# ChainBreak/denoising_diffusion_deep_fake

Hardware: AMD Instinct MI355X
Metric: training images/sec (256x256 U-Net, bs=16/GPU) (higher is better)
Workload: dtype f32; 1 GPU; d3f train_denoiser step: noise blend -> Unet(resnet34) fwd -> (MSE+1-SSIM)/2 -> bwd -> Adam, 256x256 synthetic face crops, bs=16/GPU, random-init weights, train-mode BatchNorm; image_size=256, batch_per_gpu=16, global_batch=16, parallelism=dp1, graph_step=False, adam_overlap_tail=False, adam_overlap_tail_steps=0, ranks_seen=1, csrc_digest=7380406eeae80552

## Files before the change

### denoising_diffusion_deep_fake_amd/csrc/common.h

```cpp
#pragma once
#include <hip/hip_runtime.h>
#include <stdint.h>
#include <stddef.h>
#include <stdlib.h>

namespace d3f {

typedef uint16_t bf16_t;

typedef float f32x16 __attribute__((ext_vector_type(16)));
typedef float f32x4 __attribute__((ext_vector_type(4)));
typedef __bf16 bf16x8 __attribute__((ext_vector_type(8)));

}
#ifndef D3F_F32
#define D3F_F32 0
#define D3F_BF16 1
#define D3F_F32X3 2
#endif
namespace d3f {

static inline const char* prof_knob(const char* name) {
#ifdef D3F_PROFILING
  return getenv(name);
// ... 168 lines not shown
  unsigned div_howo_mul, div_howo_shr, div_wo_mul, div_wo_shr;
  int cin_real;
  int sum2;
  int patch;
  int nets, plan_nets;
  long net_ws, net_out0, net_scale;
  int tile_bm, tile_bn;
};
__device__ __forceinline__ ConvParams conv_params_of_net(const ConvParams& pin, int net) {
  ConvParams p = pin;
  if (net != 0) {
    net_shift(p.src0, p.net_ws); net_shift(p.src1, p.net_ws); net_shift(p.w, p.net_ws);
    net_shift(p.out0, p.net_out0); net_shift(p.out1, p.net_ws);
    net_shift(p.stats, p.net_ws); net_shift(p.scale, p.net_scale); net_shift(p.shift, p.net_ws);
    net_shift(p.res, p.net_ws); net_shift(p.partial, p.net_ws);
    net_shift(p.bn_y, p.net_ws); net_shift(p.bn_coef, p.net_ws); net_shift(p.bn_partial, p.net_ws); net_shift(p.bn_a, p.net_ws);
  }
  return p;
}

struct ConvTile {
  int BM, BN;
};
int conv_igemm_plan(ConvParams& p, int dtype, bool allow_splitk = false);
size_t conv_splitk_floats(const ConvParams& p);
int conv_igemm_launch(const ConvParams& p, int dtype, hipStream_t stream);
bool conv_igemm_small_c(const ConvParams& p, int dtype);
bool conv_igemm_fast_addr(const ConvParams& p, bool smallc);
bool conv_winograd_fits(const ConvParams& p, int dtype);
bool conv_winograd_applies(const ConvParams& p, int dtype);
int conv_winograd_stat_rows(const ConvParams& p);
size_t conv_winograd_filter_floats(const ConvParams& p);
int conv_winograd_pack_launch(const float* w , float* u, int Cout, int Cin, hipStream_t stream);
int conv_winograd_launch(const ConvParams& p , hipStream_t stream);
bool conv_pres_applies(const ConvParams& p, int dtype);
void conv_pres_plan(ConvParams& p);
int conv_pres_launch(const ConvParams& p, hipStream_t stream);
bool conv_patch_applies(const ConvParams& p, int dtype);
bool conv_stem_applies(const ConvParams& p, int dtype);
bool conv_stem_bf16_applies(const ConvParams& p, int dtype);
void conv_patch_plan(ConvParams& p, int dtype);
int conv_patch_launch(const ConvParams& p, hipStream_t stream);

struct WgradParams {
  const void* dy;
  const void* src0;
  const void* src1;
  float* partial;
  unsigned dy_bytes, src0_bytes, src1_bytes;
  int B, Hv, Wv, C0, C1, H0s, W0s, shift0;
  int Ho, Wo, Cout;
  int KH, KW, stride, pad;
  int M;
  int cin_real;
  int splits;
  int chunks_per_split;
  int tiles_co, tiles_ci;
  int patch;
  double flops;
  int part;
  int cls;
  int ci_base;
  int slab_cin;
  int slab_taps;
  int Mi, Hc, Wc;
  int step_img, step_row, step_col;
// ... 106 lines not shown
```

### denoising_diffusion_deep_fake_amd/csrc/conv_winograd.hip

```cpp
#include "common.h"

#include <cstdlib>

namespace d3f {

namespace {
constexpr int WCK = 16;
constexpr int WPP = 18;
constexpr int WPB = 4;
typedef float wf32x2 __attribute__((ext_vector_type(2)));

__device__ __forceinline__ int vsw(int row, int ch) { return ch ^ ((row >> 2) & 3); }
}

bool conv_winograd_fits(const ConvParams& p, int dtype) {
  if (dtype != D3F_F32) return false;
  if (p.mode != CONV_RAW_STATS || p.par != 0 || p.KH != 3 || p.KW != 3 || p.stride != 1 || p.pad != 1 || p.C1 != 0 ||
      p.shift0 != 0 || p.zi != 0 || p.Ho != p.Hv || p.Wo != p.Wv || (p.Ho % 16) != 0 || (p.Wo % 16) != 0 ||
      (p.C0 % WCK) != 0 || (p.Cout % 64) != 0 || p.CoutPad < p.Cout)
    return false;
  if ((size_t)p.B * p.Hv * p.Wv * p.C0 * 4 >= (1ull << 31) || (size_t)16 * p.C0 * p.Cout * 4 >= (1ull << 31)) return false;
  return (long)p.B * (p.Ho / 16) * (p.Wo / 16) * (p.Cout / 64) <= 65535L * 4;
}
bool conv_winograd_applies(const ConvParams& p, int dtype) {
  static const bool off = getenv("D3F_NO_WINOGRAD") != nullptr;
  if (off || !conv_winograd_fits(p, dtype)) return false;
  const long wgs = (long)p.B * (p.Ho / 16) * (p.Wo / 16) * (p.Cout / 64) * plan_nets_for(p.plan_nets, 8);
  return wgs >= 256;
}
int conv_winograd_stat_rows(const ConvParams& p) { return p.B * (p.Ho / 16) * (p.Wo / 16); }
size_t conv_winograd_filter_floats(const ConvParams& p) { return (size_t)16 * p.C0 * p.Cout; }

__global__ __launch_bounds__(256) void winograd_pack_kernel(const float* __restrict__ w, float* __restrict__ u, int K, int C) {
  const int id = (int)blockIdx.x * 256 + (int)threadIdx.x;
  if (id >= K * C) return;
  const int k = id / C, c = id - k * C;
  const float* g = w + (long)id * 9;
  float t[4][3];
#pragma unroll
  for (int j = 0; j < 3; ++j) {
    const float g0 = g[j], g1 = g[3 + j], g2 = g[6 + j];
    t[0][j] = g0;
    t[1][j] = 0.5f * (g0 + g1 + g2);
    t[2][j] = 0.5f * (g0 - g1 + g2);
    t[3][j] = g2;
  }
  const long cstride = (long)(C / WCK) * K * WCK;
  float* dst = u + ((long)(c / WCK) * K + k) * WCK + (c % WCK);
#pragma unroll
  for (int i = 0; i < 4; ++i) {
    dst[(4 * i + 0) * cstride] = t[i][0];
    dst[(4 * i + 1) * cstride] = 0.5f * (t[i][0] + t[i][1] + t[i][2]);
    dst[(4 * i + 2) * cstride] = 0.5f * (t[i][0] - t[i][1] + t[i][2]);
    dst[(4 * i + 3) * cstride] = t[i][2];
  }
}

int conv_winograd_pack_launch(const float* w, float* u, int K, int C, hipStream_t stream) {
  D3F_CHECK((C % WCK) == 0 && K > 0 && C > 0, "winograd pack: %d filters x %d channels", K, C);
  hipLaunchKernelGGL(winograd_pack_kernel, dim3((unsigned)cdiv((long)K * C, 256)), dim3(256), 0, stream, w, u, K, C);
  D3F_HIP(hipGetLastError());
  return 0;
}

__global__ __launch_bounds__(256) void conv_winograd_kernel(const ConvParams pin) {
  chain_priority();
  const ConvParams p = conv_params_of_net(pin, (int)blockIdx.z);
  __shared__ __attribute__((aligned(16))) float P[WPP * WPP * WCK];
  __shared__ __attribute__((aligned(16))) float V[2][16 * 64 * WCK];
  const int H = p.Hv, W = p.Wv, C = p.C0, K = p.Cout;
  const int tid = threadIdx.x, lane = tid & 63, wave = tid >> 6;
  const int mt = wave >> 1, nt = wave & 1;
  const int bx = W / 16, by = H / 16;
  const int blk = blockIdx.x;
  const int x0 = (blk % bx) * 16, y0 = ((blk / bx) % by) * 16, b = blk / (bx * by);
  const int n0 = blockIdx.y * 64;
  const __amdgpu_buffer_rsrc_t rx = make_rsrc(p.src0, p.src0_bytes);
  const __amdgpu_buffer_rsrc_t ru = make_rsrc(p.w, p.w_bytes);

  f32x16 acc[16];
#pragma unroll
  for (int q = 0; q < 16; ++q)
#pragma unroll
    for (int r = 0; r < 16; ++r) acc[q][r] = 0.f;

  constexpr int NPX = (WPP * WPP * 4 + 255) / 256;
  uint4 px[NPX];
  unsigned poff[NPX];
#pragma unroll
  for (int i = 0; i < NPX; ++i) {
    const int id = tid + 256 * i, pix = id >> 2, h = id & 3;
    const int py = pix / WPP, pxx = pix - py * WPP;
    const int gy = y0 - 1 + py, gx = x0 - 1 + pxx;
    const bool ok = id < WPP * WPP * 4 && (unsigned)gy < (unsigned)H && (unsigned)gx < (unsigned)W;
    poff[i] = ok ? (unsigned)((((b * H + gy) * W + gx) * C + 4 * h) * 4) : BUF_OOB;
// ... 188 lines not shown
```

### denoising_diffusion_deep_fake_amd/csrc/engine.hip

```cpp
#include "engine.h"
#include <vector>

#include "head_act.h"

#include <cstdio>
#include <cstdlib>
#include <cstring>

namespace d3f {

constexpr int CS_PP = 16;
__global__ __launch_bounds__(256) void channel_sum_partial_kernel(const float* __restrict__ x, int C, long HW,
                                                                  float* __restrict__ partial, int nb, long net_in,
                                                                  long net_ws) {
  __shared__ float red[256];
  const int seg = blockIdx.x, c = blockIdx.y, b = (int)blockIdx.z % nb;
  if ((int)blockIdx.z >= nb) {
    net_shift(x, net_in); net_shift(partial, net_ws);
  }
  const float* __restrict__ plane = x + ((long)b * C + c) * HW;
  const long per = (HW + CS_PP - 1) / CS_PP, lo = (long)seg * per, hi = lo + per < HW ? lo + per : HW;
  float s = 0.f;
  if ((HW & 3) == 0 && (per & 3) == 0) {
    for (long i = lo + 4 * threadIdx.x; i < hi; i += 4 * 256) {
// ... 391 lines not shown
  if (streams[dev] == nullptr) {
    int least = 0, greatest = 0;
    D3F_HIP(hipDeviceGetStreamPriorityRange(&least, &greatest));
    D3F_HIP(hipStreamCreateWithPriority(&streams[dev], hipStreamNonBlocking, least));
  }
  *out = streams[dev];
  return 0;
}

int UnetEngine::ensure_streams() const {
  if (side_ != nullptr) return 0;
  if (int rc = shared_side_stream(&side_)) return rc;
  D3F_HIP(hipEventCreateWithFlags(&ev_join_, hipEventDisableTiming));
  D3F_HIP(hipEventCreateWithFlags(&ev_seg_, hipEventDisableTiming));
  D3F_HIP(hipEventCreateWithFlags(&ev_pack_in_, hipEventDisableTiming));
  D3F_HIP(hipEventCreateWithFlags(&ev_pack_done_, hipEventDisableTiming));
  D3F_HIP(hipEventCreateWithFlags(&ev_pack_mid_, hipEventDisableTiming));
  return 0;
}

bool UnetEngine::make_split(const NetIO* io, long in_delta, NetSplit* ns) const {
  if (nets <= 1) return false;
  ns->nets = nets;
  ns->ws = (long)net_ws_stride;
  ns->par = io->params;
  ns->grad = io->grads;
  ns->bn = io->bnstats;
  ns->in = in_delta;
  ns->out = io->out;
  return true;
}

int UnetEngine::pack_weights(const float* params0_, void* ws0_, hipStream_t s, const NetIO* io) const {
  D3F_CHECK((int)units.size() <= PACK_MAX_LAYERS, "pack_weights: %d layers exceed the table", (int)units.size());
  D3F_CHECK(nets == 1 || io != nullptr, "pack_weights: a pair engine needs the second network's offsets");
  static const bool sync_pack = getenv("D3F_NO_ASYNC_PACK") != nullptr;
  const bool async = !sync_pack && first_late_unit_ > 0;
  const int mid = async ? first_mid_unit_ : -1;
  auto params_of = [&](int n) { return reinterpret_cast<const float*>(reinterpret_cast<const char*>(params0_) + (n ? io->params : 0)); };
  auto ws_of = [&](int n) { return reinterpret_cast<char*>(ws0_) + (size_t)n * net_ws_stride; };
  auto part_of = [&](int ui) { return ui >= first_late_unit_ ? 2 : (mid > 0 && ui >= mid) ? 1 : 0; };
  for (int part = 0; part < 3; ++part) {
    if (part == 1 && mid <= 0) continue;
    PackTable t;
    t.n = 0;
    uint32_t blocks = 0;
    for (int ui = 0; ui < (int)units.size(); ++ui) {
      const Unit& u = units[ui];
      if (first_late_unit_ > 0 && part_of(ui) != part) continue;
      if (first_late_unit_ <= 0 && part != 0) continue;
      if (u.upfold) continue;
      const int nb = conv_pack_entry(u, u.w_off, u.wf_off, u.wd_off, true, u.need_dgrad, blocks, t.e[t.n++]);
      if (nb < 0) return nb;
      blocks += (uint32_t)nb;
    }
    hipStream_t ps = s;
    if (part >= 1 && async) {
      if (int rc = ensure_streams()) return rc;
      if (part == 1 || mid <= 0) {
        D3F_HIP(hipEventRecord(ev_pack_in_, s));
        D3F_HIP(hipStreamWaitEvent(side_, ev_pack_in_, 0));
      }
      ps = side_;
    }
    for (int n = 0; n < nets; ++n) {
      const float* params_ = params_of(n);
      char* ws = ws_of(n);
      if (t.n > 0)
        if (int rc = pack_all_launch(cdtype, params_, ws, t, (int)blocks, ps)) return rc;
      for (int ui = 0; ui < (int)units.size(); ++ui) {
        const Unit& u = units[ui];
        if (!u.wino) continue;
        if (first_late_unit_ > 0 ? part_of(ui) != part : part != 0) continue;
        if (int rc = conv_winograd_pack_launch(params_ + u.w_off, reinterpret_cast<float*>(ws + u.wu_off), u.Cout, u.Cin, ps))
          return rc;
      }
    }
    if (part == 1 && async) {
      D3F_HIP(hipEventRecord(ev_pack_mid_, side_));
      pack_mid_pending_ = true;
    }
    if (part == 2 || (first_late_unit_ <= 0 && part == 0)) {
      for (int n = 0; n < nets; ++n) {
        const float* params_ = params_of(n);
        char* ws = ws_of(n);
        for (const Unit& u : units)
          if (u.upfold)
            if (int rc = pack_up_launch(cdtype, params_ + u.w_off, u.Cout, u.C0, u.C1, ws + u.wfc_off, u.CoutPad,
                                        u.need_dgrad ? ws + u.wd4_off : nullptr, u.C0Rows,
                                        (u.need_dgrad && u.C1 > 0) ? ws + u.wds_off : nullptr, u.C1Rows, ps))
              return rc;
      }
    }
    if (part == 2 && async) {
      D3F_HIP(hipEventRecord(ev_pack_done_, side_));
      pack_pending_ = true;
    }
  }
  return 0;
}

int UnetEngine::forward(const float* params_, float* bnstats, const float* x, float* out, void* ws_,
                        int training, hipStream_t s, const NetIO* io) const {
  char* ws = reinterpret_cast<char*>(ws_);
  D3F_CHECK(nets == 1 || (io != nullptr && training), "unet: the pair engine runs train-mode passes and needs the second "
            "network's offsets");
  NetSplit split{};
  const NetSplit* ns = make_split(io, io ? io->x : 0, &split) ? &split : nullptr;
  if (int rc = nchw_to_nhwc_launch(dtype, x, ws + tensors[t_x].off, B, in_channels, H, W, tensors[t_x].C, s, ns))
    return rc;
  return forward_body(params_, bnstats, out, ws, training, s, ns);
}

int UnetEngine::forward_body(const float* params_, float* bnstats, float* out, char* ws, int training,
                             hipStream_t s, const NetSplit* ns, bool apply_act) const {
  auto T = [&](int tid) { return ws + tensors[tid].off; };
  auto coef = [&](const Unit& u) { return reinterpret_cast<float*>(ws + u.coef_off); };
  D3F_CHECK(ns == nullptr || (training && bn_sync() == nullptr), "unet: the pair engine runs train-mode passes with "
            "per-GPU BatchNorm statistics");
  if (!training) {
    BnEvalTable t;
    t.n = 0;
    for (const Unit& u : units)
      if (u.bn) {
        D3F_CHECK(t.n < PACK_MAX_LAYERS && u.coef_off % 16 == 0, "eval coefficients: table overflow");
        BnEvalEntry& e = t.e[t.n++];
// ... 594 lines not shown
```

### denoising_diffusion_deep_fake_amd/csrc/pointwise.h

```cpp
#pragma once
#include <string>

#include "common.h"
#include "philox.h"

namespace d3f {

constexpr int PACK_MAX_LAYERS = 64;

enum BnCoefRow { BN_MEAN, BN_INVSTD, BN_SCALE, BN_SHIFT, BN_K, BN_COEF_ROWS = BN_K + 3 };
inline float* bn_coef(float* block, int C, BnCoefRow row) { return block + (long)row * C; }
inline const float* bn_coef(const float* block, int C, BnCoefRow row) { return block + (long)row * C; }

struct BnEvalEntry {
  uint32_t g_off, b_off, rm_off, rv_off;
  uint32_t coef_off16;
  int32_t C;
};
struct BnEvalTable {
  int n;
  BnEvalEntry e[PACK_MAX_LAYERS];
};
int bn_eval_coeff_all_launch(const float* params, const float* bnstats, void* ws, const BnEvalTable& t,
                             hipStream_t stream);
// ... 185 lines not shown
    return true;
  }
  const float angle = s0 * q.angle_unit, scale = 1.0f + (u1 * 2.0f - 1.0f) * q.scale_span;
  const float dx = s2 * q.shift_x, dy = s3 * q.shift_y;
  sincosf(angle * q.deg2rad, &sn, &cs);
  cs = cs / scale;
  sn = sn / scale;
  const float a11 = cs, a12 = -sn * q.h_over_w, a21 = sn * q.w_over_h, a22 = cs;
  t[0] = a11, t[1] = a12, t[2] = -2.0f * (a11 * dx + a12 * dy);
  t[3] = a21, t[4] = a22, t[5] = -2.0f * (a21 * dx + a22 * dy);
  return rng_uniform24(rng_block(seed, offset, (uint32_t)b, RNG_G_APPLY).x[0]) < q.p;
}

int pool_batch_launch(const uint8_t* pool, int64_t N, const int64_t* index, float* out, int B, int H, int W,
                      const float mean[3], const float stdv[3], const float* theta, const uint8_t* apply, uint64_t seed,
                      uint64_t offset, const AffineRngParams* q, hipStream_t stream);
int pool_batch_balanced_launch(const uint8_t* pool, int64_t N, const int64_t* members, const int64_t* class_start, int Kn,
                               float* out, int64_t* index_out, int B, int H, int W, const float mean[3],
                               const float stdv[3], uint64_t seed, uint64_t offset, const AffineRngParams* q,
                               hipStream_t stream);
int balanced_index_draw_launch(const int64_t* members, const int64_t* class_start, int Kn, uint64_t seed, uint64_t offset,
                               int64_t* index_out, int B, hipStream_t stream);
__device__ __forceinline__ int64_t balanced_index_rng(uint64_t seed, uint64_t offset, int b,
                                                      const int64_t* __restrict__ members,
                                                      const int64_t* __restrict__ class_start, int Kn) {
  const Philox4 p = rng_block(seed, offset, (uint32_t)b, RNG_G_APPLY);
  const uint32_t j = (uint32_t)(((uint64_t)p.x[1] * (uint32_t)Kn) >> 32);
  const int64_t start = class_start[j], cnt = class_start[j + 1] - start;
  if (cnt <= 0 || cnt >= ((int64_t)1 << 31)) return -1;
  const int64_t m = (int64_t)(((uint64_t)p.x[2] * (uint64_t)cnt) >> 32);
  return members[start + m];
}

int pack_up_launch(int dtype, const float* w, int Cout, int C0, int C1, void* wfc, int CoutPad, void* wd4,
                   int C0Rows, void* wds, int C1Rows, hipStream_t stream);

constexpr int PACK_NT = 32;
constexpr int PACK_LDS_ROW = 288;
struct PackEntry {
  uint32_t w_off;
  uint32_t wf_off16, wd_off16;
  uint32_t block0;
  uint16_t Cout, CinReal, Cin, taps, CoutPad, Kpad, CinRows, CoutD, KpadD, has_d, CT, ctiles;
  uint16_t conv_stride;
  uint16_t has_f;
  uint16_t taps_shr, ct_log2;
  uint32_t taps_mul;
};
struct PackTable {
  int n;
  PackEntry e[PACK_MAX_LAYERS];
};
static_assert(sizeof(PackEntry) == 52, "PackTable travels as a kernel argument: keep its entries small");
int pack_all_launch(int dtype, const float* params, void* ws, const PackTable& t, int blocks,
                    hipStream_t stream);

int noise_blend_launch(const float* x, const float* noise, const float* y_uniform, float lam,
                       float* out, float* r_out, int B, long per_image, hipStream_t stream);
int noise_blend_fixed_launch(const float* x, const float* noise, const float* r, float* out, int B, long per_image,
                             hipStream_t stream);
int noise_blend_rng_launch(const float* x, uint64_t seed, uint64_t offset, float lam, float* out, float* r_out, int B,
                           long per_image, hipStream_t stream);
int noise_blend_fixed_rng_launch(const float* x, uint64_t seed, uint64_t offset, const float* r, float* out, int B,
                                 long per_image, hipStream_t stream);
int noise_blend_fixed_index_rng_launch(const float* x, uint64_t seed, uint64_t offset, const float* r,
                                       const int64_t* index, float* out, int B, long per_image, hipStream_t stream);
int noise_draw_launch(uint64_t seed, uint64_t offset, float* noise, float* y, int B, long per_image,
                      hipStream_t stream);
size_t quality_per_image_workspace_bytes(int B, int H, int W);
int quality_per_image_scatter_launch(const float* pred, const float* target, float in_min, float in_max,
                                     const int64_t* index_or_null, float* metrics, int N, void* workspace, int B, int H,
                                     int W, hipStream_t stream);
size_t l1_per_image_workspace_bytes(int B);
int l1_per_image_launch(const float* pred, const float* target, float* out, void* workspace, int B, long per_image,
                        hipStream_t stream);
constexpr int L1_PARTS = 64;
int l1_partials_launch(const float* pred, const float* target, double* partial , int B, long per_image,
                       hipStream_t stream);
__device__ __forceinline__ float l1_image_mean(const double* __restrict__ partial, int b, long per_image) {
  double s = 0.0;
  for (int i = 0; i < L1_PARTS; ++i) s += partial[(long)b * L1_PARTS + i];
  return (float)(s / (double)per_image);
}
int l1_per_image_scatter_launch(const float* pred, const float* target, const int64_t* index, float* scores, int N,
                                void* workspace, int B, long per_image, hipStream_t stream);
size_t difficulty_classes_workspace_bytes(int N);
// ... 18 lines not shown
```

### denoising_diffusion_deep_fake_amd/csrc/pointwise.hip

```cpp
#include "pointwise.h"
#include "philox.h"
#include "vec16.h"

#include <type_traits>

namespace d3f {

template <typename T>
__global__ __launch_bounds__(256) void maxpool_fwd_kernel(const T* __restrict__ in, T* __restrict__ out,
                                                          uint8_t* __restrict__ idx, int B, int H,
                                                          int W, int C, long net_ws) {
  chain_priority();
  if (blockIdx.z != 0) {
    net_shift(in, net_ws); net_shift(out, net_ws); net_shift(idx, net_ws);
  }
  constexpr int N = V16<T>::N;
  const int Ho = H / 2, Wo = W / 2, VC = C / N;
  const long total = (long)B * Ho * Wo * VC;
  for (long i = (long)blockIdx.x * 256 + threadIdx.x; i < total; i += (long)gridDim.x * 256) {
    const int cv = (int)(i % VC);
    long t = i / VC;
    const int ox = (int)(t % Wo);
    t /= Wo;
    const int oy = (int)(t % Ho);
    const int b = (int)(t / Ho);
    float best[N];
    int bi[N];
    bool first = true;
#pragma unroll
    for (int kh = 0; kh < 3; ++kh) {
      const int iy = 2 * oy - 1 + kh;
      if ((unsigned)iy >= (unsigned)H) continue;
#pragma unroll
      for (int kw = 0; kw < 3; ++kw) {
        const int ix = 2 * ox - 1 + kw;
        if ((unsigned)ix >= (unsigned)W) continue;
// ... 444 lines not shown
  if (dtype == D3F_F32)
    hipLaunchKernelGGL(nhwc_to_nchw_kernel<float>, dim3(grid_for(total)), dim3(256), 0, stream,
                       (const float*)in, out, B, C, (long)H * W, Cpad);
  else
    hipLaunchKernelGGL(nhwc_to_nchw_kernel<bf16_t>, dim3(grid_for(total)), dim3(256), 0, stream,
                       (const bf16_t*)in, out, B, C, (long)H * W, Cpad);
  D3F_HIP(hipGetLastError());
  return 0;
}

__device__ __forceinline__ int dgrad_tap_slot_to_flipped(int slot, int taps, int stride) {
  if (stride == 2 && taps == 9) return (int)((0x453718620ull >> (4 * slot)) & 15);
  return slot;
}
template <typename T, bool X3>
__device__ __forceinline__ void pack_store(T* __restrict__ base, long idx, long plane, float v) {
  if constexpr (X3) {
    const uint32_t xb = __float_as_uint(v), hb = xb & 0xffff0000u;
    const float r1 = v - __uint_as_float(hb);
    const uint32_t mb = __float_as_uint(r1) & 0xffff0000u;
    const float r2 = r1 - __uint_as_float(mb);
    base[idx] = (T)(hb >> 16);
    base[plane + idx] = (T)(mb >> 16);
    base[2 * plane + idx] = (T)(__float_as_uint(r2) >> 16);
  } else {
    base[idx] = from_f32<T>(v);
  }
}

__device__ __forceinline__ unsigned up_fwd_set(int parity, int a) {
  return parity == 0 ? (a == 0 ? 1u : 6u) : (a == 0 ? 3u : 4u);
}
__device__ __forceinline__ unsigned up_bwd_set(int u) { return u == 0 ? 4u : u == 1 ? 6u : u == 2 ? 3u : 1u; }

struct UpDiv {
  unsigned fplane[2], kc[2], c0[2], c1[2], k9[2], cd[2], k4[2];
};
template <typename T, bool X3>
__global__ __launch_bounds__(256) void pack_up_kernel(const float* __restrict__ w, int Cout, int C0, int C1,
                                                      T* __restrict__ wfc, int CoutPad, T* __restrict__ wd4,
                                                      int C0Rows, T* __restrict__ wds, int C1Rows, int CoutD,
                                                      int K9, UpDiv dv) {
  const int Cin = C0 + C1;
  const int Kc = 4 * C0 + 9 * C1, K4 = 16 * CoutD;
  const int nf = 4 * CoutPad * Kc, nd = C0Rows * K4, ns = C1Rows * K9;
  const int fplane = CoutPad * Kc;
  for (int i = (int)blockIdx.x * 256 + (int)threadIdx.x; i < nf + nd + ns; i += (int)gridDim.x * 256) {
    if (i < nf) {
      const int z = fast_div(i, dv.fplane[0], dv.fplane[1]);
      const int r = i - z * fplane;
      const int n = fast_div(r, dv.kc[0], dv.kc[1]), k = r - n * Kc;
      float v = 0.f;
      if (n < Cout) {
        if (k < 4 * C0) {
          const int ab = fast_div(k, dv.c0[0], dv.c0[1]), c = k - ab * C0;
          const unsigned sh = up_fwd_set(z >> 1, ab >> 1), sw = up_fwd_set(z & 1, ab & 1);
          const float* __restrict__ wp = w + ((long)n * Cin + c) * 9;
#pragma unroll
          for (int kh = 0; kh < 3; ++kh)
#pragma unroll
            for (int kw = 0; kw < 3; ++kw)
              if (((sh >> kh) & 1u) && ((sw >> kw) & 1u)) v += wp[kh * 3 + kw];
        } else {
          const int kk = k - 4 * C0, tap = fast_div(kk, dv.c1[0], dv.c1[1]), c1 = kk - tap * C1;
          v = w[((long)n * Cin + C0 + c1) * 9 + tap];
        }
      }
      pack_store<T, X3>(wfc + (X3 ? 3L * z * fplane : (long)z * fplane), r, fplane, v);
    } else if (i >= nf + nd) {
      const int j = i - nf - nd;
      const int c1 = fast_div(j, dv.k9[0], dv.k9[1]), k = j - c1 * K9;
      const int f = fast_div(k, dv.cd[0], dv.cd[1]), n = k - f * CoutD;
      float v = 0.f;
      if (c1 < C1 && n < Cout && f < 9) v = w[((long)n * Cin + C0 + c1) * 9 + (8 - f)];
      pack_store<T, X3>(wds, j, ns, v);
    } else {
      const int j = i - nf;
      const int c = fast_div(j, dv.k4[0], dv.k4[1]), k = j - c * K4;
      const int uv = fast_div(k, dv.cd[0], dv.cd[1]), n = k - uv * CoutD;
      float v = 0.f;
      if (c < C0 && n < Cout) {
        const unsigned sh = up_bwd_set(uv >> 2), sw = up_bwd_set(uv & 3);
        const float* __restrict__ wp = w + ((long)n * Cin + c) * 9;
#pragma unroll
        for (int kh = 0; kh < 3; ++kh)
#pragma unroll
          for (int kw = 0; kw < 3; ++kw)
            if (((sh >> kh) & 1u) && ((sw >> kw) & 1u)) v += wp[kh * 3 + kw];
      }
      pack_store<T, X3>(wd4, j, nd, v);
    }
  }
}

int pack_up_launch(int dtype, const float* w, int Cout, int C0, int C1, void* wfc, int CoutPad, void* wd4,
                   int C0Rows, void* wds, int C1Rows, hipStream_t stream) {
  const int ve = dtype == D3F_BF16 ? 8 : 4;
  const int CoutD = (int)round_up(Cout, ve);
  if (wd4 == nullptr) C0Rows = 0;
  if (wds == nullptr) C1Rows = 0;
  const int K9 = (int)round_up(9L * CoutD, dtype == D3F_BF16 ? 64 : 32);
  const long total = 4L * CoutPad * (4 * C0 + 9 * C1) + (long)C0Rows * 16 * CoutD + (long)C1Rows * K9;
  if (total == 0) return 0;
  D3F_CHECK(total < (1L << 31) - 2048L * 256, "pack_up: %ld elements exceed the 32-bit element index", total);
  UpDiv dv;
  auto setup = [](long d, unsigned (&o)[2]) { fast_div_setup((unsigned)(d > 0 ? d : 1), &o[0], &o[1]); };
  setup((long)CoutPad * (4 * C0 + 9 * C1), dv.fplane);
  setup(4 * C0 + 9 * C1, dv.kc);
  setup(C0, dv.c0);
  setup(C1, dv.c1);
  setup(K9, dv.k9);
  setup(CoutD, dv.cd);
  setup(16 * CoutD, dv.k4);
  if (dtype == D3F_F32)
    hipLaunchKernelGGL((pack_up_kernel<float, false>), dim3(grid_for(total)), dim3(256), 0, stream, w, Cout, C0, C1,
                       (float*)wfc, CoutPad, (float*)wd4, C0Rows, (float*)wds, C1Rows, CoutD, K9, dv);
  else if (dtype == D3F_F32X3)
    hipLaunchKernelGGL((pack_up_kernel<bf16_t, true>), dim3(grid_for(total)), dim3(256), 0, stream, w, Cout, C0, C1,
                       (bf16_t*)wfc, CoutPad, (bf16_t*)wd4, C0Rows, (bf16_t*)wds, C1Rows, CoutD, K9, dv);
  else
    hipLaunchKernelGGL((pack_up_kernel<bf16_t, false>), dim3(grid_for(total)), dim3(256), 0, stream, w, Cout, C0, C1,
                       (bf16_t*)wfc, CoutPad, (bf16_t*)wd4, C0Rows, (bf16_t*)wds, C1Rows, CoutD, K9, dv);
  D3F_HIP(hipGetLastError());
  return 0;
}

template <typename T, bool X3>
__global__ __launch_bounds__(256) void pack_all_kernel(const float* __restrict__ params, char* __restrict__ ws,
                                                       PackTable t) {
  __shared__ float tile[PACK_NT * (PACK_LDS_ROW + 1)];
  int l = 0;
  while (l + 1 < t.n && blockIdx.x >= t.e[l + 1].block0) ++l;
  const PackEntry e = t.e[l];
  const float* __restrict__ w = params + e.w_off;
  T* __restrict__ wf = reinterpret_cast<T*>(ws + (size_t)e.wf_off16 * 16);
  T* __restrict__ wd = reinterpret_cast<T*>(ws + (size_t)e.wd_off16 * 16);
  const int taps = e.taps, Cin = e.Cin, CinReal = e.CinReal, Cout = e.Cout, Kpad = e.Kpad, KpadD = e.KpadD,
            CoutD = e.CoutD, CT = e.CT, CoutPad = e.CoutPad, CinRows = e.CinRows;
  const int rel = (int)(blockIdx.x - e.block0);
  const int nt = rel / e.ctiles, ct = rel % e.ctiles;
  const int n0 = nt * PACK_NT, c0 = ct * CT;
  const int run = CT * taps, stride = run + 1;
  const unsigned tmul = e.taps_mul, tshr = e.taps_shr, lgct = e.ct_log2;
  constexpr int LU = 8;
  for (int i0 = threadIdx.x; i0 < PACK_NT * run; i0 += 256 * LU) {
    float v[LU];
    int dst[LU];
#pragma unroll
    for (int u = 0; u < LU; ++u) {
      const int i = i0 + u * 256;
      const int nl = fast_div(i >> lgct, tmul, tshr), r = i - nl * run;
      const int n = n0 + nl, c = c0 + fast_div(r, tmul, tshr);
      dst[u] = i < PACK_NT * run ? nl * stride + r : -1;
      const bool real = dst[u] >= 0 && n < Cout && c < CinReal;
      const float x = w[real ? (unsigned)((n * CinReal + c0) * taps + r) : 0u];
      v[u] = real ? x : 0.f;
    }
#pragma unroll
    for (int u = 0; u < LU; ++u)
      if (dst[u] >= 0) tile[dst[u]] = v[u];
  }
  __syncthreads();
  if (e.has_f) {
    for (int i = threadIdx.x; i < PACK_NT * run; i += 256) {
      const int cl = i & (CT - 1), q = i >> lgct;
      const int nl = fast_div(q, tmul, tshr), tap = q - nl * taps;
      const int n = n0 + nl, c = c0 + cl;
// ... 45 lines not shown
```

Measured before the change: 2078 images/sec.

## Batch winograd and upsample-fold weight packing into table-driven single launches

Folds the per-layer winograd filter-transform launches into the existing table-driven pack_all kernel as a new entry kind, and replaces the per-layer pack_up launches with one table-driven pack_up_all kernel per network. The new upsample pack kernel stages each 32x32 filter tile through LDS before emitting the forward, dgrad and skip layouts, instead of each element re-reading its taps from global memory. The aim is fewer kernel launches per step and less redundant global traffic during weight packing. It enlarges the kernel-argument tables, introduces 1024-thread blocks and new index-decode logic that must match the old layouts.

```diff
diff --git a/denoising_diffusion_deep_fake_amd/csrc/common.h b/denoising_diffusion_deep_fake_amd/csrc/common.h
--- a/denoising_diffusion_deep_fake_amd/csrc/common.h
+++ b/denoising_diffusion_deep_fake_amd/csrc/common.h
@@ -224,6 +224,8 @@
 int conv_winograd_stat_rows(const ConvParams& p);
 size_t conv_winograd_filter_floats(const ConvParams& p);
 int conv_winograd_pack_launch(const float* w , float* u, int Cout, int Cin, hipStream_t stream);
+struct PackEntry;
+int conv_winograd_pack_entry(long w_off, size_t wu_off, int Cout, int Cin, uint32_t block0, PackEntry& e);
 int conv_winograd_launch(const ConvParams& p , hipStream_t stream);
 bool conv_pres_applies(const ConvParams& p, int dtype);
 void conv_pres_plan(ConvParams& p);
diff --git a/denoising_diffusion_deep_fake_amd/csrc/conv_winograd.hip b/denoising_diffusion_deep_fake_amd/csrc/conv_winograd.hip
--- a/denoising_diffusion_deep_fake_amd/csrc/conv_winograd.hip
+++ b/denoising_diffusion_deep_fake_amd/csrc/conv_winograd.hip
@@ -1,4 +1,5 @@
 #include "common.h"
+#include "pointwise.h"
 
 #include <cstdlib>
 
@@ -31,36 +32,29 @@
 int conv_winograd_stat_rows(const ConvParams& p) { return p.B * (p.Ho / 16) * (p.Wo / 16); }
 size_t conv_winograd_filter_floats(const ConvParams& p) { return (size_t)16 * p.C0 * p.Cout; }
 
-__global__ __launch_bounds__(256) void winograd_pack_kernel(const float* __restrict__ w, float* __restrict__ u, int K, int C) {
-  const int id = (int)blockIdx.x * 256 + (int)threadIdx.x;
-  if (id >= K * C) return;
-  const int k = id / C, c = id - k * C;
-  const float* g = w + (long)id * 9;
-  float t[4][3];
-#pragma unroll
-  for (int j = 0; j < 3; ++j) {
-    const float g0 = g[j], g1 = g[3 + j], g2 = g[6 + j];
-    t[0][j] = g0;
-    t[1][j] = 0.5f * (g0 + g1 + g2);
-    t[2][j] = 0.5f * (g0 - g1 + g2);
-    t[3][j] = g2;
-  }
-  const long cstride = (long)(C / WCK) * K * WCK;
-  float* dst = u + ((long)(c / WCK) * K + k) * WCK + (c % WCK);
-#pragma unroll
-  for (int i = 0; i < 4; ++i) {
-    dst[(4 * i + 0) * cstride] = t[i][0];
-    dst[(4 * i + 1) * cstride] = 0.5f * (t[i][0] + t[i][1] + t[i][2]);
-    dst[(4 * i + 2) * cstride] = 0.5f * (t[i][0] - t[i][1] + t[i][2]);
-    dst[(4 * i + 3) * cstride] = t[i][2];
-  }
+static_assert(WCK == WINO_CK, "the filter transform writes the chunk size the kernel reads");
+int conv_winograd_pack_entry(long w_off, size_t wu_off, int K, int C, uint32_t block0, PackEntry& e) {
+  D3F_CHECK((C % WCK) == 0 && K > 0 && C > 0, "winograd pack: %d filters x %d channels", K, C);
+  D3F_CHECK(K < 65536 && C < 65536 && (long)K * C * 16 < (1L << 31), "winograd pack: %d filters x %d channels exceed the "
+            "packing table (extents below 65536, fewer than 2^31 elements)", K, C);
+  D3F_CHECK(w_off >= 0 && w_off <= 0xffffffffL && wu_off % 16 == 0 && (wu_off >> 4) < 0xffffffffull,
+            "winograd pack: layer out of table range");
+  e = PackEntry{};
+  e.kind = PACK_KIND_WINOGRAD;
+  e.w_off = (uint32_t)w_off;
+  e.wf_off16 = (uint32_t)(wu_off >> 4);
+  e.block0 = block0;
+  e.Cout = (uint16_t)K;
+  e.CinReal = (uint16_t)C;
+  return cdiv((long)K * C, 256);
 }
 
 int conv_winograd_pack_launch(const float* w, float* u, int K, int C, hipStream_t stream) {
-  D3F_CHECK((C % WCK) == 0 && K > 0 && C > 0, "winograd pack: %d filters x %d channels", K, C);
-  hipLaunchKernelGGL(winograd_pack_kernel, dim3((unsigned)cdiv((long)K * C, 256)), dim3(256), 0, stream, w, u, K, C);
-  D3F_HIP(hipGetLastError());
-  return 0;
+  PackTable t;
+  t.n = 1;
+  const int blocks = conv_winograd_pack_entry(0, 0, K, C, 0, t.e[0]);
+  if (blocks < 0) return blocks;
+  return pack_all_launch(D3F_F32, w, u, t, blocks, stream);
 }
 
 __global__ __launch_bounds__(256) void conv_winograd_kernel(const ConvParams pin) {
diff --git a/denoising_diffusion_deep_fake_amd/csrc/engine.hip b/denoising_diffusion_deep_fake_amd/csrc/engine.hip
--- a/denoising_diffusion_deep_fake_amd/csrc/engine.hip
+++ b/denoising_diffusion_deep_fake_amd/csrc/engine.hip
@@ -447,7 +447,6 @@
 }
 
 int UnetEngine::pack_weights(const float* params0_, void* ws0_, hipStream_t s, const NetIO* io) const {
-  D3F_CHECK((int)units.size() <= PACK_MAX_LAYERS, "pack_weights: %d layers exceed the table", (int)units.size());
   D3F_CHECK(nets == 1 || io != nullptr, "pack_weights: a pair engine needs the second network's offsets");
   static const bool sync_pack = getenv("D3F_NO_ASYNC_PACK") != nullptr;
   const bool async = !sync_pack && first_late_unit_ > 0;
@@ -457,15 +456,31 @@
   auto part_of = [&](int ui) { return ui >= first_late_unit_ ? 2 : (mid > 0 && ui >= mid) ? 1 : 0; };
   for (int part = 0; part < 3; ++part) {
     if (part == 1 && mid <= 0) continue;
+    const bool last = part == 2 || (first_late_unit_ <= 0 && part == 0);
     PackTable t;
-    t.n = 0;
-    uint32_t blocks = 0;
+    PackUpTable tu;
+    t.n = tu.n = 0;
+    uint32_t blocks = 0, ublocks = 0;
     for (int ui = 0; ui < (int)units.size(); ++ui) {
       const Unit& u = units[ui];
-      if (first_late_unit_ > 0 && part_of(ui) != part) continue;
-      if (first_late_unit_ <= 0 && part != 0) continue;
-      if (u.upfold) continue;
-      const int nb = conv_pack_entry(u, u.w_off, u.wf_off, u.wd_off, true, u.need_dgrad, blocks, t.e[t.n++]);
+      if (u.upfold) {
+        if (!last) continue;
+        D3F_CHECK(tu.n < PACK_UP_MAX_LAYERS, "pack_weights: more than %d folded layers", PACK_UP_MAX_LAYERS);
+        const bool d4 = u.need_dgrad, ds = u.need_dgrad && u.C1 > 0;
+        const int nb = pack_up_entry(cdtype, u.w_off, u.Cout, u.C0, u.C1, (int64_t)u.wfc_off, u.CoutPad, d4,
+                                     d4 ? (int64_t)u.wd4_off : 0, u.C0Rows, ds, ds ? (int64_t)u.wds_off : 0, u.C1Rows,
+                                     ublocks, tu.e[tu.n++]);
+        if (nb < 0) return nb;
+        ublocks += (uint32_t)nb;
+        continue;
+      }
+      if (first_late_unit_ > 0 ? part_of(ui) != part : part != 0) continue;
+      D3F_CHECK(t.n + (u.wino ? 2 : 1) <= PACK_MAX_LAYERS, "pack_weights: more than %d table entries", PACK_MAX_LAYERS);
+      int nb = conv_pack_entry(u, u.w_off, u.wf_off, u.wd_off, true, u.need_dgrad, blocks, t.e[t.n++]);
+      if (nb < 0) return nb;
+      blocks += (uint32_t)nb;
+      if (!u.wino) continue;
+      nb = conv_winograd_pack_entry(u.w_off, u.wu_off, u.Cout, u.Cin, blocks, t.e[t.n++]);
       if (nb < 0) return nb;
       blocks += (uint32_t)nb;
     }
@@ -478,35 +493,14 @@
       }
       ps = side_;
     }
-    for (int n = 0; n < nets; ++n) {
-      const float* params_ = params_of(n);
-      char* ws = ws_of(n);
-      if (t.n > 0)
-        if (int rc = pack_all_launch(cdtype, params_, ws, t, (int)blocks, ps)) return rc;
-      for (int ui = 0; ui < (int)units.size(); ++ui) {
-        const Unit& u = units[ui];
-        if (!u.wino) continue;
-        if (first_late_unit_ > 0 ? part_of(ui) != part : part != 0) continue;
-        if (int rc = conv_winograd_pack_launch(params_ + u.w_off, reinterpret_cast<float*>(ws + u.wu_off), u.Cout, u.Cin, ps))
-          return rc;
-      }
-    }
+    for (int n = 0; n < nets; ++n)
+      if (int rc = pack_all_launch(cdtype, params_of(n), ws_of(n), t, (int)blocks, ps)) return rc;
     if (part == 1 && async) {
       D3F_HIP(hipEventRecord(ev_pack_mid_, side_));
       pack_mid_pending_ = true;
     }
-    if (part == 2 || (first_late_unit_ <= 0 && part == 0)) {
-      for (int n = 0; n < nets; ++n) {
-        const float* params_ = params_of(n);
-        char* ws = ws_of(n);
-        for (const Unit& u : units)
-          if (u.upfold)
-            if (int rc = pack_up_launch(cdtype, params_ + u.w_off, u.Cout, u.C0, u.C1, ws + u.wfc_off, u.CoutPad,
-                                        u.need_dgrad ? ws + u.wd4_off : nullptr, u.C0Rows,
-                                        (u.need_dgrad && u.C1 > 0) ? ws + u.wds_off : nullptr, u.C1Rows, ps))
-              return rc;
-      }
-    }
+    for (int n = 0; n < nets; ++n)
+      if (int rc = pack_up_all_launch(cdtype, params_of(n), ws_of(n), tu, (int)ublocks, ps)) return rc;
     if (part == 2 && async) {
       D3F_HIP(hipEventRecord(ev_pack_done_, side_));
       pack_pending_ = true;
diff --git a/denoising_diffusion_deep_fake_amd/csrc/pointwise.h b/denoising_diffusion_deep_fake_amd/csrc/pointwise.h
--- a/denoising_diffusion_deep_fake_amd/csrc/pointwise.h
+++ b/denoising_diffusion_deep_fake_amd/csrc/pointwise.h
@@ -241,11 +241,54 @@
   return members[start + m];
 }
 
+constexpr int PACK_UP_CT = 32;
+constexpr int PACK_UP_MAX_LAYERS = 16;
+struct PackUpEntry {
+  int64_t wfc_off, wd4_off, wds_off;
+  uint32_t w_off;
+  uint32_t block0;
+  uint16_t Cout, C0, C1, CoutPad, C0Rows, C1Rows, CoutD, K9;
+  uint16_t ctiles0, ctiles1;
+};
+struct PackUpTable {
+  int n;
+  PackUpEntry e[PACK_UP_MAX_LAYERS];
+};
+int pack_up_entry(int dtype, long w_off, int Cout, int C0, int C1, int64_t wfc_off, int CoutPad, bool has_wd4,
+                  int64_t wd4_off, int C0Rows, bool has_wds, int64_t wds_off, int C1Rows, uint32_t block0, PackUpEntry& e);
+int pack_up_all_launch(int dtype, const float* params, void* ws, const PackUpTable& t, int blocks, hipStream_t stream);
 int pack_up_launch(int dtype, const float* w, int Cout, int C0, int C1, void* wfc, int CoutPad, void* wd4,
                    int C0Rows, void* wds, int C1Rows, hipStream_t stream);
 
 constexpr int PACK_NT = 32;
 constexpr int PACK_LDS_ROW = 288;
+constexpr int PACK_KIND_LAYOUT = 0, PACK_KIND_WINOGRAD = 1;
+constexpr int WINO_CK = 16;
+
+__device__ __forceinline__ void winograd_filter_transform(const float* __restrict__ w, float* __restrict__ u, int K, int C,
+                                                          int id) {
+  const int k = id / C, c = id - k * C;
+  const float* g = w + (long)id * 9;
+  float t[4][3];
+#pragma unroll
+  for (int j = 0; j < 3; ++j) {
+    const float g0 = g[j], g1 = g[3 + j], g2 = g[6 + j];
+    t[0][j] = g0;
+    t[1][j] = 0.5f * (g0 + g1 + g2);
+    t[2][j] = 0.5f * (g0 - g1 + g2);
+    t[3][j] = g2;
+  }
+  const long cstride = (long)(C / WINO_CK) * K * WINO_CK;
+  float* dst = u + ((long)(c / WINO_CK) * K + k) * WINO_CK + (c % WINO_CK);
+#pragma unroll
+  for (int i = 0; i < 4; ++i) {
+    dst[(4 * i + 0) * cstride] = t[i][0];
+    dst[(4 * i + 1) * cstride] = 0.5f * (t[i][0] + t[i][1] + t[i][2]);
+    dst[(4 * i + 2) * cstride] = 0.5f * (t[i][0] - t[i][1] + t[i][2]);
+    dst[(4 * i + 3) * cstride] = t[i][2];
+  }
+}
+
 struct PackEntry {
   uint32_t w_off;
   uint32_t wf_off16, wd_off16;
@@ -254,13 +297,15 @@
   uint16_t conv_stride;
   uint16_t has_f;
   uint16_t taps_shr, ct_log2;
+  uint16_t kind;
   uint32_t taps_mul;
 };
 struct PackTable {
   int n;
   PackEntry e[PACK_MAX_LAYERS];
 };
-static_assert(sizeof(PackEntry) == 52, "PackTable travels as a kernel argument: keep its entries small");
+static_assert(sizeof(PackEntry) == 56, "PackTable travels as a kernel argument: keep its entries small");
+static_assert(sizeof(PackTable) <= 3840 && sizeof(PackUpTable) <= 3840, "kernel arguments: 4 KB in all");
 int pack_all_launch(int dtype, const float* params, void* ws, const PackTable& t, int blocks,
                     hipStream_t stream);
 
diff --git a/denoising_diffusion_deep_fake_amd/csrc/pointwise.hip b/denoising_diffusion_deep_fake_amd/csrc/pointwise.hip
--- a/denoising_diffusion_deep_fake_amd/csrc/pointwise.hip
+++ b/denoising_diffusion_deep_fake_amd/csrc/pointwise.hip
@@ -2,6 +2,7 @@
 #include "philox.h"
 #include "vec16.h"
 
+#include <algorithm>
 #include <type_traits>
 
 namespace d3f {
@@ -512,97 +513,155 @@
   return parity == 0 ? (a == 0 ? 1u : 6u) : (a == 0 ? 3u : 4u);
 }
 __device__ __forceinline__ unsigned up_bwd_set(int u) { return u == 0 ? 4u : u == 1 ? 6u : u == 2 ? 3u : 1u; }
-
-struct UpDiv {
-  unsigned fplane[2], kc[2], c0[2], c1[2], k9[2], cd[2], k4[2];
-};
+__device__ __forceinline__ float up_tap_sum(const float* g, unsigned sh, unsigned sw) {
+  float v = 0.f;
+#pragma unroll
+  for (int kh = 0; kh < 3; ++kh)
+#pragma unroll
+    for (int kw = 0; kw < 3; ++kw)
+      if (((sh >> kh) & 1u) && ((sw >> kw) & 1u)) v += g[kh * 3 + kw];
+  return v;
+}
+
+constexpr int PACK_UP_THREADS = 1024;
 template <typename T, bool X3>
-__global__ __launch_bounds__(256) void pack_up_kernel(const float* __restrict__ w, int Cout, int C0, int C1,
-                                                      T* __restrict__ wfc, int CoutPad, T* __restrict__ wd4,
-                                                      int C0Rows, T* __restrict__ wds, int C1Rows, int CoutD,
-                                                      int K9, UpDiv dv) {
-  const int Cin = C0 + C1;
-  const int Kc = 4 * C0 + 9 * C1, K4 = 16 * CoutD;
-  const int nf = 4 * CoutPad * Kc, nd = C0Rows * K4, ns = C1Rows * K9;
-  const int fplane = CoutPad * Kc;
-  for (int i = (int)blockIdx.x * 256 + (int)threadIdx.x; i < nf + nd + ns; i += (int)gridDim.x * 256) {
-    if (i < nf) {
-      const int z = fast_div(i, dv.fplane[0], dv.fplane[1]);
-      const int r = i - z * fplane;
-      const int n = fast_div(r, dv.kc[0], dv.kc[1]), k = r - n * Kc;
-      float v = 0.f;
-      if (n < Cout) {
-        if (k < 4 * C0) {
-          const int ab = fast_div(k, dv.c0[0], dv.c0[1]), c = k - ab * C0;
-          const unsigned sh = up_fwd_set(z >> 1, ab >> 1), sw = up_fwd_set(z & 1, ab & 1);
-          const float* __restrict__ wp = w + ((long)n * Cin + c) * 9;
-#pragma unroll
-          for (int kh = 0; kh < 3; ++kh)
-#pragma unroll
-            for (int kw = 0; kw < 3; ++kw)
-              if (((sh >> kh) & 1u) && ((sw >> kw) & 1u)) v += wp[kh * 3 + kw];
-        } else {
-          const int kk = k - 4 * C0, tap = fast_div(kk, dv.c1[0], dv.c1[1]), c1 = kk - tap * C1;
-          v = w[((long)n * Cin + C0 + c1) * 9 + tap];
+__global__ __launch_bounds__(PACK_UP_THREADS) void pack_up_all_kernel(const float* __restrict__ params, char* __restrict__ ws,
+                                                          PackUpTable t) {
+  __shared__ float tile[PACK_NT * (PACK_LDS_ROW + 1)];
+  static_assert(PACK_NT == 32 && PACK_UP_CT == 32 && PACK_UP_CT * 9 == PACK_LDS_ROW, "the index decode below");
+  constexpr int CT = PACK_UP_CT, RUN = CT * 9, STRIDE = RUN + 1;
+  int l = 0;
+  while (l + 1 < t.n && blockIdx.x >= t.e[l + 1].block0) ++l;
+  const PackUpEntry e = t.e[l];
+  const int Cout = e.Cout, C0 = e.C0, C1 = e.C1, CoutPad = e.CoutPad, CoutD = e.CoutD;
+  const int Cin = C0 + C1, Kc = 4 * C0 + 9 * C1;
+  const int ctiles = e.ctiles0 + e.ctiles1;
+  const int rel = (int)(blockIdx.x - e.block0);
+  const int nt = rel / ctiles, ct = rel - nt * ctiles;
+  const bool skip = ct >= e.ctiles0;
+  const int n0 = nt * PACK_NT, c0 = (skip ? ct - e.ctiles0 : ct) * CT;
+  const int cbase = skip ? C0 : 0, Csrc = skip ? C1 : C0;
+  const float* __restrict__ w = params + e.w_off;
+  constexpr int LU = 9;
+  for (int i0 = threadIdx.x; i0 < PACK_NT * RUN; i0 += PACK_UP_THREADS * LU) {
+    float v[LU];
+    int dst[LU];
+#pragma unroll
+    for (int u = 0; u < LU; ++u) {
+      const int i = i0 + u * PACK_UP_THREADS;
+      const int nl = i / RUN, r = i - nl * RUN;
+      const int n = n0 + nl, c = c0 + r / 9;
+      dst[u] = i < PACK_NT * RUN ? nl * STRIDE + r : -1;
+      const bool real = dst[u] >= 0 && n < Cout && c < Csrc;
+      const float x = w[real ? (unsigned)((n * Cin + cbase + c0) * 9 + r) : 0u];
+      v[u] = real ? x : 0.f;
+    }
+#pragma unroll
+    for (int u = 0; u < LU; ++u)
+      if (dst[u] >= 0) tile[dst[u]] = v[u];
+  }
+  __syncthreads();
+  T* __restrict__ wfc = reinterpret_cast<T*>(ws + e.wfc_off);
+  const long fplane = (long)CoutPad * Kc, zstep = X3 ? 3 * fplane : fplane;
+  if (!skip) {
+    for (int i = threadIdx.x; i < 16 * PACK_NT * CT; i += PACK_UP_THREADS) {
+      const int cl = i & 31, nl = (i >> 5) & 31, ab = (i >> 10) & 3, z = i >> 12;
+      const int n = n0 + nl, c = c0 + cl;
+      if (n < CoutPad && c < C0) {
+        const float v = up_tap_sum(tile + nl * STRIDE + cl * 9, up_fwd_set(z >> 1, ab >> 1), up_fwd_set(z & 1, ab & 1));
+        pack_store<T, X3>(wfc + z * zstep, (long)n * Kc + ab * C0 + c, fplane, v);
+      }
+    }
+    if (e.C0Rows) {
+      T* __restrict__ wd4 = reinterpret_cast<T*>(ws + e.wd4_off);
+      const long K4 = 16L * CoutD, nd = e.C0Rows * K4;
+      for (int i = threadIdx.x; i < 16 * CT * PACK_NT; i += PACK_UP_THREADS) {
+        const int nl = i & 31, cl = (i >> 5) & 31, uv = i >> 10;
+        const int n = n0 + nl, c = c0 + cl;
+        if (c < e.C0Rows && n < CoutD) {
+          const float v = up_tap_sum(tile + nl * STRIDE + cl * 9, up_bwd_set(uv >> 2), up_bwd_set(uv & 3));
+          pack_store<T, X3>(wd4, c * K4 + uv * CoutD + n, nd, v);
         }
       }
-      pack_store<T, X3>(wfc + (X3 ? 3L * z * fplane : (long)z * fplane), r, fplane, v);
-    } else if (i >= nf + nd) {
-      const int j = i - nf - nd;
-      const int c1 = fast_div(j, dv.k9[0], dv.k9[1]), k = j - c1 * K9;
-      const int f = fast_div(k, dv.cd[0], dv.cd[1]), n = k - f * CoutD;
-      float v = 0.f;
-      if (c1 < C1 && n < Cout && f < 9) v = w[((long)n * Cin + C0 + c1) * 9 + (8 - f)];
-      pack_store<T, X3>(wds, j, ns, v);
-    } else {
-      const int j = i - nf;
-      const int c = fast_div(j, dv.k4[0], dv.k4[1]), k = j - c * K4;
-      const int uv = fast_div(k, dv.cd[0], dv.cd[1]), n = k - uv * CoutD;
-      float v = 0.f;
-      if (c < C0 && n < Cout) {
-        const unsigned sh = up_bwd_set(uv >> 2), sw = up_bwd_set(uv & 3);
-        const float* __restrict__ wp = w + ((long)n * Cin + c) * 9;
-#pragma unroll
-        for (int kh = 0; kh < 3; ++kh)
-#pragma unroll
-          for (int kw = 0; kw < 3; ++kw)
-            if (((sh >> kh) & 1u) && ((sw >> kw) & 1u)) v += wp[kh * 3 + kw];
-      }
-      pack_store<T, X3>(wd4, j, nd, v);
-    }
-  }
+    }
+  } else {
+    for (int i = threadIdx.x; i < 9 * PACK_NT * CT; i += PACK_UP_THREADS) {
+      const int cl = i & 31, nl = (i >> 5) & 31, tap = i >> 10;
+      const int n = n0 + nl, c1 = c0 + cl;
+      if (n < CoutPad && c1 < C1) {
+        const float v = tile[nl * STRIDE + cl * 9 + tap];
+        const long idx = (long)n * Kc + 4 * C0 + tap * C1 + c1;
+#pragma unroll
+        for (int z = 0; z < 4; ++z) pack_store<T, X3>(wfc + z * zstep, idx, fplane, v);
+      }
+    }
+    if (e.C1Rows) {
+      T* __restrict__ wds = reinterpret_cast<T*>(ws + e.wds_off);
+      const long K9 = e.K9, ns = e.C1Rows * K9;
+      for (int i = threadIdx.x; i < 9 * CT * PACK_NT; i += PACK_UP_THREADS) {
+        const int nl = i & 31, cl = (i >> 5) & 31, f = i >> 10;
+        const int n = n0 + nl, c1 = c0 + cl;
+        if (c1 < e.C1Rows && n < CoutD)
+          pack_store<T, X3>(wds, c1 * K9 + f * CoutD + n, ns, tile[nl * STRIDE + cl * 9 + (8 - f)]);
+      }
+      if (nt == 0) {
+        const int k0 = 9 * CoutD, tail = (int)K9 - k0;
+        for (int i = threadIdx.x; i < CT * tail; i += PACK_UP_THREADS) {
+          const int c1 = c0 + i / tail;
+          if (c1 < e.C1Rows) pack_store<T, X3>(wds, c1 * K9 + k0 + i % tail, ns, 0.f);
+        }
+      }
+    }
+  }
+}
+
+int pack_up_entry(int dtype, long w_off, int Cout, int C0, int C1, int64_t wfc_off, int CoutPad, bool has_wd4,
+                  int64_t wd4_off, int C0Rows, bool has_wds, int64_t wds_off, int C1Rows, uint32_t block0, PackUpEntry& e) {
+  const int ve = dtype == D3F_BF16 ? 8 : 4;
+  const int CoutD = (int)round_up(Cout, ve);
+  if (!has_wd4) C0Rows = 0;
+  if (!has_wds) C1Rows = 0;
+  const long K9 = round_up(9L * CoutD, dtype == D3F_BF16 ? 64 : 32);
+  const long total = 4L * CoutPad * (4L * C0 + 9L * C1) + (long)C0Rows * 16 * CoutD + (long)C1Rows * K9;
+  const long extent = std::max({(long)Cout, (long)C0, (long)C1, (long)CoutPad, (long)C0Rows, (long)C1Rows, K9});
+  D3F_CHECK(Cout >= 0 && C0 >= 0 && C1 >= 0 && CoutPad >= Cout && extent < 65536 && total < (1L << 31) &&
+                (long)Cout * (C0 + C1) * 9 < (1L << 31),
+            "pack_up: the layer exceeds the packing table (extents below 65536, fewer than 2^31 elements): extent %ld, "
+            "%ld packed elements", extent, total);
+  D3F_CHECK(w_off >= 0 && w_off <= 0xffffffffL, "pack_up: layer out of table range");
+  e = PackUpEntry{};
+  e.wfc_off = wfc_off; e.wd4_off = wd4_off; e.wds_off = wds_off;
+  e.w_off = (uint32_t)w_off;
+  e.block0 = block0;
+  e.Cout = (uint16_t)Cout; e.C0 = (uint16_t)C0; e.C1 = (uint16_t)C1; e.CoutPad = (uint16_t)CoutPad;
+  e.C0Rows = (uint16_t)C0Rows; e.C1Rows = (uint16_t)C1Rows; e.CoutD = (uint16_t)CoutD; e.K9 = (uint16_t)K9;
+  e.ctiles0 = (uint16_t)cdiv(std::max(C0, C0Rows), PACK_UP_CT);
+  e.ctiles1 = (uint16_t)cdiv(std::max(C1, C1Rows), PACK_UP_CT);
+  if (total == 0) return 0;
+  return (e.ctiles0 + e.ctiles1) * cdiv(std::max(CoutPad, CoutD), PACK_NT);
+}
+
+int pack_up_all_launch(int dtype, const float* params, void* ws, const PackUpTable& t, int blocks, hipStream_t stream) {
+  if (t.n == 0 || blocks == 0) return 0;
+  if (dtype == D3F_F32)
+    hipLaunchKernelGGL((pack_up_all_kernel<float, false>), dim3(blocks), dim3(PACK_UP_THREADS), 0, stream, params, (char*)ws, t);
+  else if (dtype == D3F_F32X3)
+    hipLaunchKernelGGL((pack_up_all_kernel<bf16_t, true>), dim3(blocks), dim3(PACK_UP_THREADS), 0, stream, params, (char*)ws, t);
+  else
+    hipLaunchKernelGGL((pack_up_all_kernel<bf16_t, false>), dim3(blocks), dim3(PACK_UP_THREADS), 0, stream, params, (char*)ws, t);
+  D3F_HIP(hipGetLastError());
+  return 0;
 }
 
 int pack_up_launch(int dtype, const float* w, int Cout, int C0, int C1, void* wfc, int CoutPad, void* wd4,
                    int C0Rows, void* wds, int C1Rows, hipStream_t stream) {
-  const int ve = dtype == D3F_BF16 ? 8 : 4;
-  const int CoutD = (int)round_up(Cout, ve);
-  if (wd4 == nullptr) C0Rows = 0;
-  if (wds == nullptr) C1Rows = 0;
-  const int K9 = (int)round_up(9L * CoutD, dtype == D3F_BF16 ? 64 : 32);
-  const long total = 4L * CoutPad * (4 * C0 + 9 * C1) + (long)C0Rows * 16 * CoutD + (long)C1Rows * K9;
-  if (total == 0) return 0;
-  D3F_CHECK(total < (1L << 31) - 2048L * 256, "pack_up: %ld elements exceed the 32-bit element index", total);
-  UpDiv dv;
-  auto setup = [](long d, unsigned (&o)[2]) { fast_div_setup((unsigned)(d > 0 ? d : 1), &o[0], &o[1]); };
-  setup((long)CoutPad * (4 * C0 + 9 * C1), dv.fplane);
-  setup(4 * C0 + 9 * C1, dv.kc);
-  setup(C0, dv.c0);
-  setup(C1, dv.c1);
-  setup(K9, dv.k9);
-  setup(CoutD, dv.cd);
-  setup(16 * CoutD, dv.k4);
-  if (dtype == D3F_F32)
-    hipLaunchKernelGGL((pack_up_kernel<float, false>), dim3(grid_for(total)), dim3(256), 0, stream, w, Cout, C0, C1,
-                       (float*)wfc, CoutPad, (float*)wd4, C0Rows, (float*)wds, C1Rows, CoutD, K9, dv);
-  else if (dtype == D3F_F32X3)
-    hipLaunchKernelGGL((pack_up_kernel<bf16_t, true>), dim3(grid_for(total)), dim3(256), 0, stream, w, Cout, C0, C1,
-                       (bf16_t*)wfc, CoutPad, (bf16_t*)wd4, C0Rows, (bf16_t*)wds, C1Rows, CoutD, K9, dv);
-  else
-    hipLaunchKernelGGL((pack_up_kernel<bf16_t, false>), dim3(grid_for(total)), dim3(256), 0, stream, w, Cout, C0, C1,
-                       (bf16_t*)wfc, CoutPad, (bf16_t*)wd4, C0Rows, (bf16_t*)wds, C1Rows, CoutD, K9, dv);
-  D3F_HIP(hipGetLastError());
-  return 0;
+  PackUpTable t;
+  t.n = 1;
+  auto off = [&](const void* p) { return p ? (int64_t)((intptr_t)p - (intptr_t)wfc) : (int64_t)0; };
+  const int blocks = pack_up_entry(dtype, 0, Cout, C0, C1, 0, CoutPad, wd4 != nullptr, off(wd4), C0Rows, wds != nullptr,
+                                   off(wds), C1Rows, 0, t.e[0]);
+  if (blocks < 0) return blocks;
+  return pack_up_all_launch(dtype, w, wfc, t, blocks, stream);
 }
 
 template <typename T, bool X3>
@@ -613,6 +672,12 @@
   while (l + 1 < t.n && blockIdx.x >= t.e[l + 1].block0) ++l;
   const PackEntry e = t.e[l];
   const float* __restrict__ w = params + e.w_off;
+  if (e.kind == PACK_KIND_WINOGRAD) {
+    const int id = (int)(blockIdx.x - e.block0) * 256 + (int)threadIdx.x;
+    if (id < (int)e.Cout * (int)e.CinReal)
+      winograd_filter_transform(w, reinterpret_cast<float*>(ws + (size_t)e.wf_off16 * 16), e.Cout, e.CinReal, id);
+    return;
+  }
   T* __restrict__ wf = reinterpret_cast<T*>(ws + (size_t)e.wf_off16 * 16);
   T* __restrict__ wd = reinterpret_cast<T*>(ws + (size_t)e.wd_off16 * 16);
   const int taps = e.taps, Cin = e.Cin, CinReal = e.CinReal, Cout = e.Cout, Kpad = e.Kpad, KpadD = e.KpadD,
```

New measurement: 2090 images/sec (median of 6 runs). No clear change (+0.6%).
